# KrainskiL/CGE.jl

Measured on AMD Instinct MI355X. Metric: edge_alpha_evals_per_sec, higher is better.
Workload: dtype f64

## Files before the change

### cge.jl_amd/api.py

```python
from __future__ import annotations

import atexit
import ctypes as C
import os
import sys
import weakref

import numpy as np

from .args import _SplitRule

_HERE = os.path.dirname(os.path.abspath(__file__))
_LIB_PATH = os.path.join(_HERE, "csrc", "build", "libcge_hip.so")
_lib = None

CGE_OK = 0
_CODES = {-1: "AssertionError", -2: "ErrorException: Trying to split homogenous cluster",
          -3: "ErrorException: Unexpected empty cluster generated", -4: "HIP error / no GPU",
          -5: "collective hook failed", -6: "out of memory", -7: "bad argument"}


class CGEError(RuntimeError):
    def __init__(self, code, msg=""):
        super().__init__(f"{_CODES.get(code, 'error')} (code {code}){': ' + msg if msg else ''}")
# ... 817 lines not shown
        T, d = off.size - 1, self.d
        assert T >= 1 and off[0] == 0 and off[-1] == ids.size
        if z is not None:
            z = _f64(z)
            assert z.shape == ids.shape
        rc, nlow, children = np.zeros(T, dtype=np.int32), np.zeros(T, dtype=np.int32), np.full(ids.size, -1, dtype=np.int32)
        vlow, vhigh, cmeans = np.zeros(T), np.zeros(T), np.full((T, 2, d), np.nan)
        route, ties = np.zeros(T, dtype=np.int32), C.c_int32()
        self._check(self.L.cge_group_cut_test(self.h, _p(ids), _p(off), C.c_int64(T), C.c_int(int(method)), _p(z),
                                              C.c_int(1 if force_generic else 0), _p(rc), _p(nlow), _p(children), _p(vlow),
                                              _p(vhigh), _p(cmeans), _p(route), C.byref(ties)))
        return {"rc": rc, "nlow": nlow, "children": children, "vlow": vlow, "vhigh": vhigh, "cmeans": cmeans, "route": route,
                "ties": ties.value}

    def diameter_bounds_test(self, v_to_l, N, lcomm, C_, pass_):
        v2l, lc = _i64(v_to_l), _i64(lcomm)
        w = int(C_) if C_ >= 32 else int(N)
        P, ref, mean = np.zeros((N, w)), np.zeros((w, self.d)), np.zeros(self.d)
        nref, ran = C.c_int64(), C.c_int()
        self._check(self.L.cge_diameter_bounds_test(self.h, _p(v2l), C.c_int64(N), _p(lc), C.c_int64(C_), C.c_int(pass_), _p(P),
                                                    C.byref(nref), C.byref(ran), _p(ref), _p(mean)))
        assert nref.value == w
        return P, ran.value, ref, mean

    def landmark_graph_test(self, v_to_l, N, directed=False, wedge_form=0, part=0, nparts=1, aggregate=False, wedges=True,
                            positive=None, degrees=False, world=0):
        v2l = _i64(v_to_l)
        N = int(N)
        io, out = LandmarkGraphIO(), {}
        io.v2l, io.N, io.directed, io.wedge_form = v2l.ctypes.data, N, int(bool(directed)), int(wedge_form)
        io.part, io.nparts, io.world = int(part), int(nparts), int(world)

        def want(key, shape, dtype=np.float64):
            out[key] = np.full(shape, -1 if dtype != np.float64 else np.nan, dtype=dtype)
            setattr(io, key, out[key].ctypes.data)

        if aggregate:
            d = getattr(self, "d", 1)
            want("lemb", (N, d)), want("lweight", N), want("dii", N), want("lcomm", N, np.int32)
        positive = bool(wedges) if positive is None else positive
        if wedges:
            want("wedges", (N, N))
        if positive:
            want("positive", 1, np.int64)
        if degrees:
            want("deg_out", N), want("deg_in", N), want("star", N, np.int32)
# ... 334 lines not shown
                cap = count.value
                continue
            self._check(rc)
            break
        return [(comm[l], int(nc[l]), float(q[l]), int(rounds[l])) for l in range(count.value)]

    def ecg(self, members=16, w_min=0.05, seed=0, final_level=-1, edge_weights=False):
        args = EcgArgs(int(members), float(w_min), int(seed), int(final_level))
        out = np.zeros(self.n, dtype=np.int64)
        w = np.zeros(self.m) if edge_weights else None
        nc, q, q_ecg = C.c_int64(), C.c_double(), C.c_double()
        self._check(self.L.cge_ecg(self.h, C.byref(args), _p(out), C.byref(nc), C.byref(q), C.byref(q_ecg), _p(w) if edge_weights else None))
        return (out, nc.value, q.value, q_ecg.value) + ((w,) if edge_weights else ())

    def ecg_members_test(self, members=16, seed=0):
        K = int(members)
        mem = np.zeros((max(K, 1), self.n), dtype=np.int64)
        nc, rounds, q = np.zeros(max(K, 1), dtype=np.int64), np.zeros(max(K, 1), dtype=np.int64), np.zeros(max(K, 1))
        core = np.zeros(self.n, dtype=np.int32)
        self._check(self.L.cge_ecg_members_test(self.h, C.c_int64(K), C.c_int64(int(seed)), _p(mem), _p(nc), _p(rounds), _p(q), _p(core)))
        return mem, nc, rounds, q, core.astype(bool)

    _TEST_OPTIONS = ("louvain_wave_len", "fit_persistent_test_delay", "fit_persistent_test_timeout", "test_bvec_plain", "test_rss2_one_kernel",
                     "exact_resident_limit", "test_eig_roles", "fit_dir_tiles")

    def set_option(self, key, value):
        if key in self._TEST_OPTIONS:
            self._check(self.L.cge_set_test_option(self.h, key.encode(), C.c_int64(int(value))))
            return
        self._check(self.L.cge_set_option(self.h, key.encode(), C.c_int64(int(value))))

    def get_stat(self, key):
        v = C.c_int64()
        self._check(self.L.cge_get_stat(self.h, key.encode(), C.byref(v)))
        return v.value

    def last_diameter(self):
        import struct

        hi = struct.unpack("d", struct.pack("q", self.get_stat("diameter_bits")))[0]
        return hi, {1: "brute", 2: "pruned"}.get(self.get_stat("diameter_path"), "none"), \
            self.get_stat("diameter_candidate_pairs"), self.get_stat("diameter_candidate_tiles")

    def profile_enable(self, on=True):
        self._check(self.L.cge_profile_enable(self.h, C.c_int(int(on))))

    def profile_select(self, names=()):
# ... 126 lines not shown
```

### cge.jl_amd/csrc/capi.cpp

```cpp
#include "common.hpp"
#include "../../include/cge_hip_testing.h"

void flush_timers(cge_ctx *c) {
    for (auto &kv : c->timers) {
        for (auto &pr : kv.second.pending) {
            float ms = 0.f;
            (void)hipEventSynchronize(pr.second);
            if (hipEventElapsedTime(&ms, pr.first, pr.second) == hipSuccess) kv.second.total_ms += ms;
            c->event_pool.push_back(pr.first);
            c->event_pool.push_back(pr.second);
        }
        kv.second.pending.clear();
    }
}
template <class Map>
static int key_names(const Map &m, char *buf, int64_t buf_len) {
    std::string s;
    for (auto &kv : m) s += (s.empty() ? "" : ",") + kv.first;
    snprintf(buf, (size_t)buf_len, "%s", s.c_str());
    return CGE_OK;
}

extern "C" {

// ... 300 lines not shown
    if (is("fit_persistent")) return ranged(c->opt_fit_persistent, 0, 2);
    if (is("pow_exp2")) return flag(c->opt_pow_exp2);
    if (is("shard_runsplit")) return ranged(c->opt_shard_forced, 0, 2);
    if (is("shard_samples")) return ranged(c->opt_shard_samples, 0, 2);
    if (is("exact_relabel")) return flag(c->opt_exact_relabel);
    if (is("bvec_blocks")) return flag(c->opt_bvec_blocks);
    if (is("wedges_reduce_scatter")) return flag(c->opt_wedges_rs);
    if (is("fit_fused")) return flag(c->opt_fit_fused);
    if (is("shard_ingest")) return flag(c->opt_shard_ingest);
    if (is("shard_rows")) return flag(c->opt_shard_rows);
    if (is("landmark_edges")) return flag(c->opt_landmark_edges);
    if (is("exact_packed")) return ranged(c->opt_exact_packed, 0, 1);
    if (is("exact_packed_directed")) return ranged(c->opt_exact_packed_directed, 0, 2);
    if (is("fit_max_iterations")) return ranged(c->opt_fit_max_iters, 1, INT64_MAX);
    if (is("ecg_group")) return ranged(c->opt_ecg_group, 0, 64);
    return CGE_E_ARG;
}
int cge_set_test_option(void *ctx, const char *key, int64_t value) {
    cge_ctx *c = (cge_ctx *)ctx;
    if (!c || !key) return CGE_E_ARG;
    if (!strcmp(key, "test_bvec_plain")) { c->opt_test_bvec_plain = value != 0; return CGE_OK; }
    if (!strcmp(key, "test_rss2_one_kernel")) { c->opt_test_rss2_one_kernel = value != 0; return CGE_OK; }
    if (!strcmp(key, "test_eig_roles") && value >= 0 && value <= 3) { c->opt_test_eig_roles = (int)value; return CGE_OK; }
    if (!strcmp(key, "fit_persistent_test_delay") && value >= 0 && value <= 100000) { c->opt_fit_test_delay = (int)value; return CGE_OK; }
    if (!strcmp(key, "fit_persistent_test_timeout")) { c->opt_fit_test_timeout = value != 0; return CGE_OK; }
    if (!strcmp(key, "louvain_wave_len") && value >= -2 && value <= INT32_MAX) { c->opt_test_louvain_wave_len = value; return CGE_OK; }
    if (!strcmp(key, "fit_dir_tiles")) { c->opt_test_fit_dir_tiles = value != 0; return CGE_OK; }
    if (!strcmp(key, "exact_resident_limit") && value >= 0) { c->opt_test_resident_limit = (double)value; return CGE_OK; }
    return CGE_E_ARG;
}
int cge_get_stat(cge_ctx *c, const char *key, int64_t *value) {
    if (!c || !key || !value) return CGE_E_ARG;
    if (!strcmp(key, "landmarks")) *value = c->lm_ready ? c->N : 0;
    else if (!strcmp(key, "diameter_path")) *value = c->stat_diameter_path;
    else if (!strcmp(key, "diameter_candidate_pairs")) *value = c->stat_cand_pairs;
    else if (!strcmp(key, "diameter_candidate_tiles")) *value = c->stat_cand_tiles;
    else if (!strcmp(key, "diameter_refs")) *value = c->stat_nref;
    else if (!strcmp(key, "diameter_bound_pass")) *value = c->stat_bound_pass;
    else if (!strcmp(key, "diameter_arg_i")) *value = c->stat_hi_i + 1;
    else if (!strcmp(key, "diameter_arg_j")) *value = c->stat_hi_j + 1;
    else if (!strcmp(key, "fit_persistent_alphas")) *value = c->stat_fit_persistent;
    else if (!strcmp(key, "fit_iterations")) *value = c->stat_fit_iters;
    else if (!strcmp(key, "exact_packed")) *value = c->stat_exact_packed;
    else if (!strcmp(key, "exact_matrix_bytes")) *value = c->stat_exact_matrix_bytes;
    else if (!strcmp(key, "fit_fused_alphas")) *value = c->stat_fit_fused;
    else if (!strcmp(key, "fit_persistent_fallbacks")) *value = c->stat_fit_fallbacks;
// ... 133 lines not shown
    host_group_stats_test(c, ids, task_row_off, T, side, mean_in, mean, sw, cov, vec, z, sums);
    CGE_CATCH(c)
}

int cge_group_cut_test(void *ctx, const int32_t *ids, const int32_t *task_row_off, int64_t T, int method, const double *z, int force_generic,
                       int32_t *rc, int32_t *nlow, int32_t *children, double *vlow, double *vhigh, double *cmeans, int32_t *route,
                       int32_t *ties) {
    cge_ctx *c = (cge_ctx *)ctx;
    if (!c || !ids || !task_row_off || T <= 0 || !rc || !nlow || !children || !vlow || !vhigh || !cmeans || !route || !ties) return CGE_E_ARG;
    CGE_TRY_ON_DEVICE(c)
    host_group_cut_test(c, ids, task_row_off, T, method, z, force_generic, rc, nlow, children, vlow, vhigh, cmeans, route, ties);
    CGE_CATCH(c)
}

int cge_diameter_bounds_test(void *ctx, const int64_t *v2l, int64_t N, const int64_t *lcomm, int64_t C, int pass, double *P,
                             int64_t *nref, int *pass_ran, double *ref_points, double *mean) {
    cge_ctx *c = (cge_ctx *)ctx;
    if (!c || !v2l || !lcomm || !P || !nref || !pass_ran || N <= 0 || C <= 0 || pass < 0 || pass > 2) return CGE_E_ARG;
    CGE_TRY_ON_DEVICE(c)
    host_diameter_bounds_test(c, v2l, N, lcomm, C, pass, P, nref, pass_ran, ref_points, mean);
    CGE_CATCH(c)
}

int cge_landmark_graph_test(void *ctx, cge_landmark_graph_io *io) {
    cge_ctx *c = (cge_ctx *)ctx;
    if (!c || !io || !io->v2l || io->N <= 0 || io->wedge_form < 0 || io->wedge_form > 2) return CGE_E_ARG;
    CGE_TRY_ON_DEVICE(c)
    host_landmark_graph_test(c, io);
    CGE_CATCH(c)
}
int cge_wedge_geometry_test(int64_t N, int weighted, int64_t n_chunks, int *applies, int *rshift, int *colbits, int64_t *ntile,
                            int64_t *lds_pass1, int64_t *lds_pass2) {
    if (!applies || !rshift || !colbits || !ntile || !lds_pass1 || !lds_pass2) return CGE_E_ARG;
    WedgeGeometry G;
    *applies = k_wedge_geometry(N, weighted ? 8 : 4, n_chunks, &G) ? 1 : 0;
    if (!*applies) return CGE_OK;
    *rshift = G.rshift; *colbits = G.colbits; *ntile = G.ntile;
    *lds_pass1 = (int64_t)G.lds1; *lds_pass2 = (int64_t)G.lds2;
    return CGE_OK;
}

int cge_pow_test(void *ctx, const double *x, int64_t n, double alpha, int method, double *out) {
    cge_ctx *c = (cge_ctx *)ctx;
    if (!c || !x || !out || n <= 0) return CGE_E_ARG;
    CGE_TRY(c)
    k_pow_test(c, x, n, alpha, method, out);
// ... 143 lines not shown
```

### cge.jl_amd/csrc/common.hpp

```cpp
#pragma once
#include <hip/hip_runtime.h>

#include <algorithm>
#include <atomic>
#include <chrono>
#include <condition_variable>
#include <functional>
#include <mutex>
#include <thread>
#include <cstdint>
#include <cstdio>
#include <cstdlib>
#include <cstring>
#include <map>
#include <memory>
#include <string>
#include <vector>

#include "../../include/cge_hip.h"

typedef int64_t i64;
typedef int32_t i32;

struct MaxRec {
// ... 331 lines not shown
    DevBuf<double> sw_fused_pw;
    DevBuf<char> sw_fused_epi;
    int opt_fit_fused = 1;
    i64 stat_fit_fused = 0;
    DevBuf<double> batch_scal, batch_vectB, batch_jspart, batch_flow;
    PinBuf<double> batch_pin;
    i64 stat_fit_batched_launches = 0, stat_fit_batched_alphas = 0;
    DevBuf<i32> sw_rl_order, sw_rl_comm;
    DevBuf<double> sw_rl_emb, sw_rl_vec, sw_rl_T;
    DevBuf<int> fp_flags;
    PinBuf<double> pin_scal;
    hipEvent_t sweep_ev[2] = {nullptr, nullptr};
    int opt_pow_exp2 = 1;
    i64 pow_logs_N = 0;
    bool pow_logs_upper = false;
    i64 pow_logs_blocked_N = 0;
    DevBuf<double> sw_Lh;
    DevBuf<float> sw_Ll;
    bool opt_exact_relabel = true;
    int opt_shard_samples = 1;
    int opt_shard_forced = 1;
    int opt_test_rss2_one_kernel = 0;
    int opt_test_eig_roles = 0;
    i64 opt_test_louvain_wave_len = -2;
    int opt_ecg_group = 0;
    i64 stat_ecg_groups = 0, stat_ecg_member_rounds = 0, stat_ecg_peel_rounds = 0, stat_ecg_levels = 0;
    int opt_test_bvec_plain = 0;
    int opt_fit_persistent = 0;
    i64 opt_fit_max_iters = 2000000;
    int opt_fit_test_timeout = 0;
    int opt_fit_test_delay = 0;
    i64 stat_lm_batches = 0, stat_lm_rows = 0, stat_lm_splits = 0;
    DevBuf<int> cut_ties;
    i64 stat_fit_persistent = 0;
    i64 stat_fit_iters = 0;
    bool fit_persistent_broken = false;
    i64 stat_fit_fallbacks = 0;
    int fit_fallback_streak = 0;
    i64 fit_skip_sweeps = 0;
    DevBuf<i32> sw_cm_off, sw_cm_mem, sw_cm_pos;
    DevBuf<double> sw_zeros, sw_zsum;
    DevBuf<MaxRec> mp_recs;
    DevBuf<i64> mp_count;
    DevBuf<int2> nt_pairs, nt_tiles;
    DevBuf<i32> nt_idx;
    DevBuf<double> nt_out, nt_rows;
// ... 473 lines not shown
void k_js(cge_ctx *c, const double *vC, const double *vB, i64 len, i64 C, int directed, int mode ,
          double *out, double *partials = nullptr);
void k_auc_landmark(cge_ctx *c, const double *Ta, const double *Tb, const i32 *v2l, const double *vw_orig,
                    const double *lweight, const i32 *pi, const i32 *pj, const i32 *ni, const i32 *nj,
                    const double *dpos, const double *dneg, const double *wts, i64 S, double alpha, double *out2, double *partials = nullptr);
void k_auc_exact(cge_ctx *c, const double *GD, const double *Ta, const double *Tb, i64 N, const i32 *pi,
                 const i32 *pj, const i32 *ni, const i32 *nj, const double *wts, i64 S, double *out2, double *partials = nullptr,
                 bool packed = false);
void k_gather_i32(cge_ctx *c, const i32 *arr, const i32 *idx, i64 S, i32 *out);
void k_mark_edge_hits(cge_ctx *c, const i32 *src, const i32 *dst, i64 m, int directed, const uint64_t *table,
                      i64 table_size, i32 *hit);

void host_runsplit(cge_ctx *c, const i64 *cl_flat, const i64 *cl_off, i64 ncl, i64 nland, i64 forced, int method,
                   std::vector<i64> &group_ids , bool want_index = false);
void host_eig_top(const double *A, i64 d, double *v);
void host_group_stats_test(cge_ctx *c, const i32 *ids, const i32 *task_row_off, i64 T, const unsigned char *side, const double *mean_in,
                           double *mean, double *sw, double *cov, double *vec, double *z, double *sums);
void host_group_cut_test(cge_ctx *c, const i32 *ids, const i32 *task_row_off, i64 T, int method, const double *z, int force_generic,
                         i32 *rc, i32 *nlow, i32 *children, double *vlow, double *vhigh, double *cmeans, i32 *route, i32 *ties);
double host_diameter_brute(cge_ctx *c, int part, int nparts, i64 *ai, i64 *aj);
double host_diameter_landmarks(cge_ctx *c, const double *lemb, const double *lweight, const std::vector<i32> &lcomm, i64 C, i64 N);
void host_diameter_bounds_test(cge_ctx *c, const i64 *v2l, i64 N, const i64 *lcomm1, i64 C, int pass, double *P, i64 *nref_out,
                               int *pass_ran, double *ref_out, double *mean_out);
struct cge_landmark_graph_io;
void host_landmark_graph_test(cge_ctx *c, cge_landmark_graph_io *io);
#define CGE_TILE_DOUBLES 4096
__host__ __device__ inline i64 cge_upper_tile(i64 I, i64 J, i64 Nt) { return I * Nt - I * (I - 1) / 2 + (J - I); }
__host__ __device__ inline int cge_tile_slot(int r, int q) {
    const int lane = 8 * (r >> 3) + (q >> 3), a = r & 7, b = q & 7;
    return ((4 * a + (b >> 1)) * 64 + lane) * 2 + (b & 1);
}
__host__ __device__ inline i64 cge_packed_index(i64 i, i64 j, i64 Nt) {
    if ((i >> 6) > (j >> 6)) { const i64 s = i; i = j; j = s; }
    return cge_upper_tile(i >> 6, j >> 6, Nt) * CGE_TILE_DOUBLES + cge_tile_slot((int)(i & 63), (int)(j & 63));
}
__host__ __device__ inline void cge_upper_tile_of(i64 t, i64 Nt, i64 &I, i64 &J) {
    const double bb = 2.0 * (double)Nt + 1.0;
    I = (i64)((bb - sqrt(bb * bb - 8.0 * (double)t)) * 0.5);
    if (I < 0) I = 0;
    if (I > Nt - 1) I = Nt - 1;
    while (I + 1 < Nt && (I + 1) * Nt - (I + 1) * I / 2 <= t) I++;
    while (I > 0 && I * Nt - I * (I - 1) / 2 > t) I--;
    J = I + (t - (I * Nt - I * (I - 1) / 2));
}
__host__ __device__ inline uint64_t cge_sm64(uint64_t x) {
    x += 0x9e3779b97f4a7c15ULL;
// ... 118 lines not shown
```

### cge.jl_amd/csrc/diameter_host.cpp

```cpp
#include <algorithm>
#include <cmath>
#include <functional>
#include <limits>

#include "common.hpp"

namespace {
struct ExactBest {
    double hi = -1.0;
    i64 i = 0, j = 0;
    void offer(double v, i64 a, i64 b) {
        if (a > b) std::swap(a, b);
        if (v > hi || (v == hi && (a < i || (a == i && b < j)))) { hi = v; i = a; j = b; }
    }
};
struct SideStream {
    cge_ctx *c;
    explicit SideStream(cge_ctx *c_) : c(c_) { std::swap(c->stream, c->copy_stream); }
    ~SideStream() { std::swap(c->stream, c->copy_stream); }
};
}

static double gram_delta(i64 dpad, double rmax) { return (double)(8 * dpad + 32) * 2.220446049250313e-16 * rmax; }

// ... 560 lines not shown
        for (i64 q = mem_off[a]; q < mem_off[a + 1]; q++)
            for (i64 k = 0; k < d; k++) mu[a * d + k] += X[(i64)mem[q] * d + k];
        for (i64 k = 0; k < d; k++) mu[a * d + k] /= (double)cnt;
    }
    DevBuf<double> dmu, dlw;
    dmu.ensure((size_t)N * d);
    dlw.ensure(N);
    HIP_CHECK(hipMemcpyAsync(dmu.p, mu.data(), sizeof(double) * N * d, hipMemcpyHostToDevice, st));
    HIP_CHECK(hipMemcpyAsync(dlw.p, lw.data(), sizeof(double) * N, hipMemcpyHostToDevice, st));
    HIP_CHECK(hipStreamSynchronize(st));
    struct KeepOption { int &ref; int val; ~KeepOption() { ref = val; } } keep{c->opt_diameter_f32, c->opt_diameter_f32};
    c->opt_diameter_f32 = pass;
    DmPrep S;
    if (!dm_prepare(c, dmu.p, dlw.p, lc, C, N, mem_off, mem, S, [](const char *) {}))
        CGE_THROW(CGE_E_ARG, "diameter bounds: no landmark index");
    dm_bound_pass(c, S, N, 0, 1);
    HIP_CHECK(hipMemcpyAsync(P, c->Pm.p, sizeof(double) * (size_t)(N * S.nref), hipMemcpyDeviceToHost, st));
    if (ref_out) HIP_CHECK(hipMemcpyAsync(ref_out, S.mu_ref, sizeof(double) * (size_t)(S.nref * d), hipMemcpyDeviceToHost, st));
    if (mean_out) HIP_CHECK(hipMemcpyAsync(mean_out, c->gmean.p, sizeof(double) * d, hipMemcpyDeviceToHost, st));
    HIP_CHECK(hipStreamSynchronize(st));
    *nref_out = S.nref;
    *pass_ran = c->stat_bound_pass;
}
```

### cge.jl_amd/csrc/kernels_dist.hip

```cpp
#include "common.hpp"
#include <type_traits>
#include "mfma_tile.hpp"

#define WAVE 64

#define DT 64
#define DK 16
__device__ __forceinline__ void tile_dist2(const double *__restrict__ emb, i64 N, i64 d, i64 i0, i64 j0, int ty, int tx,
                                           double (*As)[DK + 1], double (*Bs)[DK + 1], double acc[4][4]) {
#pragma unroll
    for (int a = 0; a < 4; a++)
#pragma unroll
        for (int b = 0; b < 4; b++) acc[a][b] = 0.0;
    for (i64 k0 = 0; k0 < d; k0 += DK) {
        __syncthreads();
        for (int e = threadIdx.x; e < DT * DK; e += 256) {
            const int r = e / DK, kk = e % DK;
            const i64 k = k0 + kk;
            As[r][kk] = (i0 + r < N && k < d) ? emb[(i0 + r) * d + k] : 0.0;
            Bs[r][kk] = (j0 + r < N && k < d) ? emb[(j0 + r) * d + k] : 0.0;
        }
        __syncthreads();
        const int kmax = (int)min((i64)DK, d - k0);
        for (int kk = 0; kk < kmax; kk++) {
// ... 535 lines not shown
                            const i64 r0 = i0 + wr * 64 + a * 32 + 16 * h;
                            double v = -1e300;
#pragma unroll
                            for (int gg = 0; gg < 2; gg++)
#pragma unroll
                                for (int j = 0; j < 4; j++)
                                {
                            const float af = acc[a][b][4 * (2 * h + gg) + j];
                            v = fmax(v, (af - af == 0.f) ? rns[r0 + 8 * gg + 4 * lh + j] * e1 - 2.0 * (double)af : 1e300);
                        }
                            v = fmax(v, __shfl_xor(v, 32));
                            if (lh == 0) G[(r0 >> 4) * ldm + col] = fmax(v + mn, 0.0);
                        }
                }
            }
            __syncthreads();
        }
    }
}

typedef __bf16 bf8v __attribute__((ext_vector_type(8)));
typedef short s8v __attribute__((ext_vector_type(8)));
#define PB_APAD 8
#define PB_T 512
template <int NKS>
__global__ __launch_bounds__(PB_T) void pcent_bf16_kernel(const unsigned short *__restrict__ Xb, const double *__restrict__ rns,
                                                          i64 lds_rows, const unsigned short *__restrict__ Mb,
                                                          const double *__restrict__ mnorm, i64 ldm,
                                                          const i32 *__restrict__ sub_land, i64 nref,
                                                          unsigned long long *__restrict__ P, i64 I0, i64 I1, double e1,
                                                          int diag ) {
    extern __shared__ __attribute__((aligned(16))) unsigned short ldsb[];
    constexpr i64 KP = 16 * NKS;
    constexpr int LDA = (int)KP + PB_APAD;
    unsigned short *Ah = ldsb, *Al = Ah + (size_t)128 * LDA, *Bh = Al + (size_t)128 * LDA, *Bl = Bh + (size_t)128 * LDA;
    double *gmax = reinterpret_cast<double *>(Bl + (size_t)128 * LDA);
    const int tid = threadIdx.x, wave = tid >> 6, lane = tid & 63;
    const int wr = wave >> 1, wc = wave & 1, l32 = lane & 31, lh = lane >> 5;
    const i64 nTJ = ldm / 128;
    constexpr int apieces = (int)(KP / 8);
    const int arow = tid >> 5, apc = tid & 31;
    const bool aact = apc < 2 * apieces;
    const int apl = aact && apc >= apieces ? 1 : 0, akk = 8 * (apc - apl * apieces);
    auto fetch = [&](const unsigned short *base, i64 rows_ld, i64 r0, uint4 (&v)[8]) {
#pragma unroll
        for (int it = 0; it < 8; it++)
// ... 76 lines not shown
            __syncthreads();
            if (!(diag & 1) && tid < 128) {
                const i64 col = J * 128 + tid;
                double cur = 0.0;
                int curland = -1;
#pragma unroll
                for (int gq = 0; gq < 8; gq++) {
                    const int land = sub_land[(i0 >> 4) + gq];
                    const double v = gmax[gq * 128 + tid];
                    if (land != curland) {
                        if (curland >= 0 && col < nref) atomicMax(&P[(i64)curland * nref + col], (unsigned long long)__double_as_longlong(cur));
                        curland = land;
                        cur = v;
                    } else
                        cur = fmax(cur, v);
                }
                if (curland >= 0 && col < nref) atomicMax(&P[(i64)curland * nref + col], (unsigned long long)__double_as_longlong(cur));
            }
            if (more_cols) stash(Bh, Bl, bv);
            __syncthreads();
        }
    }
}
__global__ void pcent_groups_kernel(const double *__restrict__ G, const i32 *__restrict__ soff, i64 ldm, i64 N,
                                    double *__restrict__ P) {
    const i64 a = blockIdx.x;
    const i32 g0 = soff[a] >> 4, g1 = soff[a + 1] >> 4;
    for (i64 col = threadIdx.x; col < N; col += blockDim.x) {
        double v = 0.0;
        for (i32 g = g0; g < g1; g++) v = fmax(v, G[(i64)g * ldm + col]);
        P[a * N + col] = v;
    }
}

__global__ __launch_bounds__(256, 2) void pair_list_kernel(const double *__restrict__ Xs,
                                                           const double *__restrict__ rns, i64 lds_rows, i64 npos,
                                                           i64 dpad, const int2 *__restrict__ tiles, i64 ntiles,
                                                           MaxRec *__restrict__ recs) {
    extern __shared__ __attribute__((aligned(16))) double lds[];
    const int tid = threadIdx.x, wave = tid >> 6, lane = tid & 63;
    const int wr = wave >> 1, wc = wave & 1, lr = lane & 15, lk = lane >> 4, c2 = lane * 2;
    const i64 nchunk = dpad / MP_BK;
    double best = -1.0;
    i64 best_i = 0, best_j = 0;
    for (i64 t = blockIdx.x; t < ntiles; t += gridDim.x) {
        const i64 i0 = tiles[t].x, j0 = tiles[t].y;
// ... 99 lines not shown
    ScopedKernelTimer t(c, "pcent");
    const i64 nTI = lds_rows / 128, I0 = nTI * part / nparts, I1 = nTI * (part + 1) / nparts;
    const i64 ntiles = (I1 - I0) * (ldm / 128);
    const double e1 = 1.0 + 1.01 * (double)(dpad + 3) * 5.9604644775390625e-08;
    if (ntiles > 0 && dpad <= 128) {
        cge_allow_lds((const void *)pcent_f32_rowres_kernel, 160 * 1024);
        const size_t lds = ((size_t)dpad * 128 + 2 * PF_BK * 128) * sizeof(float);
        hipLaunchKernelGGL(pcent_f32_rowres_kernel, dim3((unsigned)std::min<i64>(I1 - I0, 512)), dim3(256), lds, c->stream, Xs32, rns,
                           lds_rows, Ms32, mnorm, ldm, N, dpad, c->pc_groups.p, I0, I1, e1);
    } else if (ntiles > 0)
        hipLaunchKernelGGL(pcent_f32_kernel, dim3((unsigned)std::min<i64>(ntiles, 2048)), dim3(256), PF_LDS_BYTES, c->stream,
                           Xs32, rns, lds_rows, Ms32, mnorm, ldm, N, dpad, c->pc_groups.p, I0, I1, e1);
    hipLaunchKernelGGL(pcent_groups_kernel, dim3((unsigned)n_land), dim3(256), 0, c->stream, c->pc_groups.p, soff, ldm, N, P);
}

bool k_pcent_bf16_applies(i64 dpad) { return (dpad + 31) / 32 * 32 <= 128; }
void k_pcent_bf16(cge_ctx *c, const unsigned short *Xb, const double *rns, i64 lds_rows, const unsigned short *Mb,
                  const double *mnorm, i64 ldm, i64 n_land, i64 N, i64 KP, const i32 *sub_land, double *P, int part, int nparts) {
    HIP_CHECK(hipMemsetAsync(P, 0, sizeof(double) * n_land * N, c->stream));
    ScopedKernelTimer t(c, "pcent");
    const i64 nTI = lds_rows / 128, I0 = nTI * part / nparts, I1 = nTI * (part + 1) / nparts;
    const double e1 = 1.0 + 1.05 * (3.0 * (double)(KP + 2) * 1.1920928955078125e-07 + 3.2 * 1.52587890625e-05);
    if (I1 > I0) {
        const size_t lds = (size_t)4 * 128 * (KP + PB_APAD) * sizeof(unsigned short) + (size_t)8 * 128 * sizeof(double);
        const int pb_diag = 0;
#define PB_GO(NKS)                                                                                                         \
    do {                                                                                                                   \
        auto kern = pcent_bf16_kernel<NKS>;                                                                                 \
        cge_allow_lds((const void *)kern, 160 * 1024); \
        hipLaunchKernelGGL(kern, dim3((unsigned)std::min<i64>(I1 - I0, 256)), dim3(PB_T), lds, c->stream, Xb, rns, lds_rows, Mb, \
                           mnorm, ldm, sub_land, N, reinterpret_cast<unsigned long long *>(P), I0, I1, e1, pb_diag);        \
    } while (0)
        if (KP == 32) PB_GO(2);
        else if (KP == 64) PB_GO(4);
        else if (KP == 96) PB_GO(6);
        else PB_GO(8);
#undef PB_GO
    }
}

void k_pair_list(cge_ctx *c, const double *Xs, const double *rns, i64 lds_rows, i64 npos, i64 dpad, const int2 *tiles,
                 i64 ntiles, double *best_val, i64 *best_i, i64 *best_j, std::vector<double> *wg_best) {
    c->mp_recs.ensure(MP_NWG);
    MaxRec *recs = c->mp_recs.p;
    const int nwg = (int)std::max<i64>(1, std::min<i64>(ntiles, MP_NWG));
    {
        ScopedKernelTimer t(c, "pair_list");
        hipLaunchKernelGGL(pair_list_kernel, dim3(nwg), dim3(256), MP_LDS_BYTES, c->stream, Xs, rns, lds_rows, npos,
                           dpad, tiles, ntiles, recs);
    }
    best_of_recs(c, recs, nwg, best_val, best_i, best_j, wg_best);
}

void k_max_pair_tile_list(i64 ldn, int part, int nparts, const std::vector<double> &wg, double thr, std::vector<int2> &out) {
// ... 25 lines not shown
    HIP_CHECK(hipStreamSynchronize(c->stream));
    return (i64)h;
}

__global__ __launch_bounds__(256) void bound_select_kernel(const double *__restrict__ Q, const i32 *__restrict__ lref,
                                                           const double *__restrict__ rd2, i64 N, i64 nref, double L,
                                                           BoundRec *__restrict__ list, i64 cap,
                                                           unsigned long long *__restrict__ count) {
    const i64 total = N * N, stride = (i64)gridDim.x * blockDim.x;
    for (i64 e = (i64)blockIdx.x * blockDim.x + threadIdx.x; e < total; e += stride) {
        const i64 a = e / N, b = e - a * N;
        if (b < a) continue;
        const i64 ra = lref[a], rb = lref[b];
        const double qaa = Q[a * nref + ra], qbb = Q[b * nref + rb];
        const double pre = Q[a * nref + rb] + Q[b * nref + ra] + 2.0 * sqrt(qaa * qbb);
        if (pre * (1.0 + 1e-9) + 1e-9 < L) continue;
        const double Bv = pre - rd2[ra * nref + rb] * (1.0 - 1e-9);
        if (Bv * (1.0 + 1e-9) + 1e-9 >= L) {
            const unsigned long long idx = atomicAdd(count, 1ULL);
            if ((i64)idx < cap) list[idx] = BoundRec{Bv, (i32)a, (i32)b};
        }
    }
}
__global__ __launch_bounds__(256) void ref_dist2_fm_kernel(const double *__restrict__ Ms, i64 nref, i64 dpad, i64 ldm,
                                                           double *__restrict__ rd2) {
    const i64 a = blockIdx.x;
    for (i64 b = threadIdx.x; b < nref; b += blockDim.x) {
        double s = 0.0;
#pragma unroll 8
        for (i64 k = 0; k < dpad; k++) {
            const double df = Ms[k * ldm + a] - Ms[k * ldm + b];
            s += df * df;
        }
        rd2[a * nref + b] = s;
    }
}
__global__ __launch_bounds__(256) void comm_max_kernel(const double *__restrict__ Q, const i32 *__restrict__ ref_off,
                                                       const i32 *__restrict__ ref_mem, i64 nref, double *__restrict__ Mx) {
    const i64 ca = blockIdx.x;
    const i32 b = ref_off[ca], e = ref_off[ca + 1];
    for (i64 r = threadIdx.x; r < nref; r += blockDim.x) {
        double v = 0.0;
        for (i32 t = b; t < e; t++) v = fmax(v, Q[(i64)ref_mem[t] * nref + r]);
        Mx[ca * nref + r] = v;
    }
}
__global__ __launch_bounds__(256) void comm_pairs_kernel(const double *__restrict__ Mx, const double *__restrict__ rd2, i64 C,
                                                         double L, int2 *__restrict__ plist, unsigned *__restrict__ pcount) {
    const i64 total = C * C, stride = (i64)gridDim.x * blockDim.x;
    for (i64 e = (i64)blockIdx.x * blockDim.x + threadIdx.x; e < total; e += stride) {
        const i64 ca = e / C, cb = e - ca * C;
        if (cb < ca) continue;
        const double pre = Mx[ca * C + cb] + Mx[cb * C + ca] + 2.0 * sqrt(Mx[ca * C + ca] * Mx[cb * C + cb]);
        if (pre * (1.0 + 1e-9) + 1e-9 < L) continue;
        const double Bv = pre - rd2[ca * C + cb] * (1.0 - 1e-9);
        if (Bv * (1.0 + 1e-9) + 1e-9 >= L) plist[atomicAdd(pcount, 1u)] = make_int2((int)ca, (int)cb);
    }
// ... 7 lines not shown
    for (unsigned q = blockIdx.x; q < np; q += gridDim.x) {
        const i64 ca = plist[q].x, cb = plist[q].y;
        const i32 a0 = ref_off[ca], na = ref_off[ca + 1] - a0, b0 = ref_off[cb], nb = ref_off[cb + 1] - b0;
        const double r2 = rd2[ca * nref + cb] * (1.0 - 1e-9);
        for (i64 e = threadIdx.x; e < (i64)na * nb; e += blockDim.x) {
            const i64 ia = e / nb, ib = e - ia * nb;
            i64 a = ref_mem[a0 + ia], b = ref_mem[b0 + ib];
            if (ca == cb && b < a) continue;
            i64 ra = ca, rb = cb;
            if (b < a) { const i64 t = a; a = b; b = t; ra = cb; rb = ca; }
            const double qaa = Q[a * nref + ra], qbb = Q[b * nref + rb];
            const double pre = Q[a * nref + rb] + Q[b * nref + ra] + 2.0 * sqrt(qaa * qbb);
            if (pre * (1.0 + 1e-9) + 1e-9 < L) continue;
            const double Bv = pre - r2;
            if (Bv * (1.0 + 1e-9) + 1e-9 >= L) {
                const unsigned long long idx = atomicAdd(count, 1ULL);
                if ((i64)idx < cap) list[idx] = BoundRec{Bv, (i32)a, (i32)b};
            }
        }
    }
}
void k_ref_dist2_fm(cge_ctx *c, const double *Ms_fm, i64 nref, i64 dpad, i64 ldm) {
    c->mp_rd2.ensure((size_t)nref * nref);
    hipLaunchKernelGGL(ref_dist2_fm_kernel, dim3((unsigned)nref), dim3(256), 0, c->stream, Ms_fm, nref, dpad, ldm, c->mp_rd2.p);
}
i64 k_bound_select(cge_ctx *c, const double *Q, const i32 *lref, i64 N, i64 nref, double L, BoundRec *list, i64 cap,
                   const i32 *ref_off, const i32 *ref_mem) {
    c->mp_count.ensure(2);
    HIP_CHECK(hipMemsetAsync(c->mp_count.p, 0, 2 * sizeof(i64), c->stream));
    ScopedKernelTimer tm(c, "bound_select");
    if (ref_off && ref_mem) {
        c->mp_commax.ensure((size_t)nref * nref);
        c->mp_plist.ensure((size_t)nref * (nref + 1) / 2);
        hipLaunchKernelGGL(comm_max_kernel, dim3((unsigned)nref), dim3(256), 0, c->stream, Q, ref_off, ref_mem, nref, c->mp_commax.p);
        hipLaunchKernelGGL(comm_pairs_kernel, dim3(grid_for(nref * nref, 256)), dim3(256), 0, c->stream, c->mp_commax.p, c->mp_rd2.p,
                           nref, L, c->mp_plist.p, reinterpret_cast<unsigned *>(c->mp_count.p + 1));
        hipLaunchKernelGGL(bound_expand_kernel, dim3(2048), dim3(256), 0, c->stream, Q, c->mp_rd2.p, ref_off, ref_mem, nref, L,
                           c->mp_plist.p, reinterpret_cast<const unsigned *>(c->mp_count.p + 1), list, cap,
                           reinterpret_cast<unsigned long long *>(c->mp_count.p));
    } else
        hipLaunchKernelGGL(bound_select_kernel, dim3(grid_for(N * N, 256)), dim3(256), 0, c->stream, Q, lref, c->mp_rd2.p, N,
                           nref, L, list, cap, reinterpret_cast<unsigned long long *>(c->mp_count.p));
    i64 cnt = 0;
    HIP_CHECK(hipMemcpyAsync(&cnt, c->mp_count.p, sizeof(i64), hipMemcpyDeviceToHost, c->stream));
    HIP_CHECK(hipStreamSynchronize(c->stream));
    return cnt;
}
// ... 208 lines not shown
```

### include/cge_hip_testing.h

```cpp
#ifndef CGE_HIP_TESTING_H
#define CGE_HIP_TESTING_H
#include <stdint.h>
#ifdef __cplusplus
extern "C" {
#endif
int cge_host_eig_top(const double *A, int64_t d, double *v);
int cge_batch_pack_test(const int64_t *N, int64_t K, int cus, int32_t *group_of);
int cge_fit_dir_geometry_test(int64_t N, int cus, int *applies, int *G, int *NW, int *NSB);
int cge_fit_slots_test(int64_t N, int directed, int64_t out[5]);
int cge_batch_pack_dir_test(const int64_t *N, int64_t K, int cus, int32_t *group_of);
int cge_host_pos_draw(int64_t seed, int64_t stream_id, int64_t S, int64_t m, int64_t *pos_idx);
int cge_group_eig(void *ctx, const double *A, int64_t T, int64_t d, double *v);
int cge_group_stats_test(void *ctx, const int32_t *ids, const int32_t *task_row_off, int64_t T, const uint8_t *side, const double *mean_in,
                         double *mean, double *sw, double *cov, double *vec, double *z, double *sums);
int cge_group_cut_test(void *ctx, const int32_t *ids, const int32_t *task_row_off, int64_t T, int method, const double *z, int force_generic,
                       int32_t *rc, int32_t *nlow, int32_t *children, double *vlow, double *vhigh, double *cmeans, int32_t *route,
                       int32_t *ties);
int cge_diameter_bounds_test(void *ctx, const int64_t *v2l, int64_t N, const int64_t *lcomm, int64_t C, int pass, double *P,
                             int64_t *nref, int *pass_ran, double *ref_points, double *mean);
typedef struct cge_landmark_graph_io {
    const int64_t *v2l;
    int64_t N;
    int32_t directed, wedge_form;
    int64_t part, nparts, world;
    double *lemb, *lweight, *dii;
    int32_t *lcomm;
    double *wedges;
    int64_t *positive;
    double *deg_out, *deg_in;
    int32_t *star;
    double *deg_block, *u_deg_out, *u_deg_in;
    int32_t *u_star;
    int64_t n_chunks, ntile;
    int32_t form_ran, rshift, colbits, pad;
} cge_landmark_graph_io;
int cge_landmark_graph_test(void *ctx, cge_landmark_graph_io *io);
int cge_wedge_geometry_test(int64_t N, int weighted, int64_t n_chunks, int *applies, int *rshift, int *colbits, int64_t *ntile,
                            int64_t *lds_pass1, int64_t *lds_pass2);
int cge_pow_test(void *ctx, const double *x, int64_t n, double alpha, int method, double *out);
#define CGE_VECT_B_GUARD 64
typedef struct cge_vect_b_problem {
    const double *GD, *Ta, *Tb;
// ... 108 lines not shown
```

Baseline: 11.96 billion.

## Add register-resident B-tile pcent kernel and tiled reference distance kernel

Adds a pcent_bf16 kernel variant that keeps the reference (B) fragments in registers per wave across many row tiles, with a double-buffered prefetch of A tiles through LDS. It is selected by default when ldm is at least 384. The reference pairwise-distance kernel is also rewritten as a 32x32 shared-memory tiled kernel instead of one block per row. Both aim to cut repeated global/LDS reads of the reference matrix, at the cost of higher register pressure and a separate code path. The change also adds test hooks for selecting the pcent form and for reference distances.

```diff
diff --git a/cge.jl_amd/api.py b/cge.jl_amd/api.py
--- a/cge.jl_amd/api.py
+++ b/cge.jl_amd/api.py
@@ -863,6 +863,14 @@
                                                     C.byref(nref), C.byref(ran), _p(ref), _p(mean)))
         assert nref.value == w
         return P, ran.value, ref, mean
+
+    def ref_dist2_test(self, refs):
+        refs = _f64(refs)
+        assert refs.ndim == 2 and refs.shape[1] == self.d
+        nref = refs.shape[0]
+        rd2, mean = np.zeros((nref, nref)), np.zeros(self.d)
+        self._check(self.L.cge_ref_dist2_test(self.h, _p(refs), C.c_int64(nref), _p(rd2), _p(mean)))
+        return rd2, mean
 
     def landmark_graph_test(self, v_to_l, N, directed=False, wedge_form=0, part=0, nparts=1, aggregate=False, wedges=True,
                             positive=None, degrees=False, world=0):
@@ -1243,7 +1251,7 @@
         return mem, nc, rounds, q, core.astype(bool)
 
     _TEST_OPTIONS = ("louvain_wave_len", "fit_persistent_test_delay", "fit_persistent_test_timeout", "test_bvec_plain", "test_rss2_one_kernel",
-                     "exact_resident_limit", "test_eig_roles", "fit_dir_tiles")
+                     "exact_resident_limit", "test_eig_roles", "fit_dir_tiles", "test_pcent_form")
 
     def set_option(self, key, value):
         if key in self._TEST_OPTIONS:
diff --git a/cge.jl_amd/csrc/capi.cpp b/cge.jl_amd/csrc/capi.cpp
--- a/cge.jl_amd/csrc/capi.cpp
+++ b/cge.jl_amd/csrc/capi.cpp
@@ -346,6 +346,7 @@
     if (!strcmp(key, "test_bvec_plain")) { c->opt_test_bvec_plain = value != 0; return CGE_OK; }
     if (!strcmp(key, "test_rss2_one_kernel")) { c->opt_test_rss2_one_kernel = value != 0; return CGE_OK; }
     if (!strcmp(key, "test_eig_roles") && value >= 0 && value <= 3) { c->opt_test_eig_roles = (int)value; return CGE_OK; }
+    if (!strcmp(key, "test_pcent_form") && value >= 0 && value <= 2) { c->opt_test_pcent_form = (int)value; return CGE_OK; }
     if (!strcmp(key, "fit_persistent_test_delay") && value >= 0 && value <= 100000) { c->opt_fit_test_delay = (int)value; return CGE_OK; }
     if (!strcmp(key, "fit_persistent_test_timeout")) { c->opt_fit_test_timeout = value != 0; return CGE_OK; }
     if (!strcmp(key, "louvain_wave_len") && value >= -2 && value <= INT32_MAX) { c->opt_test_louvain_wave_len = value; return CGE_OK; }
@@ -525,6 +526,14 @@
     CGE_CATCH(c)
 }
 
+int cge_ref_dist2_test(void *ctx, const double *refs, int64_t nref, double *rd2, double *mean) {
+    cge_ctx *c = (cge_ctx *)ctx;
+    if (!c || !refs || !rd2 || nref <= 0) return CGE_E_ARG;
+    CGE_TRY_ON_DEVICE(c)
+    host_ref_dist2_test(c, refs, nref, rd2, mean);
+    CGE_CATCH(c)
+}
+
 int cge_landmark_graph_test(void *ctx, cge_landmark_graph_io *io) {
     cge_ctx *c = (cge_ctx *)ctx;
     if (!c || !io || !io->v2l || io->N <= 0 || io->wedge_form < 0 || io->wedge_form > 2) return CGE_E_ARG;
diff --git a/cge.jl_amd/csrc/common.hpp b/cge.jl_amd/csrc/common.hpp
--- a/cge.jl_amd/csrc/common.hpp
+++ b/cge.jl_amd/csrc/common.hpp
@@ -377,6 +377,7 @@
     int opt_shard_forced = 1;
     int opt_test_rss2_one_kernel = 0;
     int opt_test_eig_roles = 0;
+    int opt_test_pcent_form = 0;
     i64 opt_test_louvain_wave_len = -2;
     int opt_ecg_group = 0;
     i64 stat_ecg_groups = 0, stat_ecg_member_rounds = 0, stat_ecg_peel_rounds = 0, stat_ecg_levels = 0;
@@ -896,6 +897,7 @@
 double host_diameter_landmarks(cge_ctx *c, const double *lemb, const double *lweight, const std::vector<i32> &lcomm, i64 C, i64 N);
 void host_diameter_bounds_test(cge_ctx *c, const i64 *v2l, i64 N, const i64 *lcomm1, i64 C, int pass, double *P, i64 *nref_out,
                                int *pass_ran, double *ref_out, double *mean_out);
+void host_ref_dist2_test(cge_ctx *c, const double *refs, i64 nref, double *rd2, double *mean_out);
 struct cge_landmark_graph_io;
 void host_landmark_graph_test(cge_ctx *c, cge_landmark_graph_io *io);
 #define CGE_TILE_DOUBLES 4096
diff --git a/cge.jl_amd/csrc/diameter_host.cpp b/cge.jl_amd/csrc/diameter_host.cpp
--- a/cge.jl_amd/csrc/diameter_host.cpp
+++ b/cge.jl_amd/csrc/diameter_host.cpp
@@ -606,3 +606,21 @@
     *nref_out = S.nref;
     *pass_ran = c->stat_bound_pass;
 }
+
+void host_ref_dist2_test(cge_ctx *c, const double *refs, i64 nref, double *rd2, double *mean_out) {
+    const i64 d = c->d, dpad = c->dpad;
+    if (!c->Xr.p || c->n <= 0 || d <= 0) CGE_THROW(CGE_E_ARG, "reference distances: embedding not resident");
+    hipStream_t st = c->stream;
+    const i64 ldm = (nref + 127) / 128 * 128;
+    DevBuf<double> dref;
+    dref.ensure((size_t)nref * d);
+    HIP_CHECK(hipMemcpyAsync(dref.p, refs, sizeof(double) * nref * d, hipMemcpyHostToDevice, st));
+    HIP_CHECK(hipStreamSynchronize(st));
+    c->Ms.ensure((size_t)ldm * dpad);
+    c->mnorm.ensure(ldm);
+    k_gather_centre_fm(c, dref.p, nullptr, c->gmean.p, c->Ms.p, c->mnorm.p, nref, d, ldm, dpad, nullptr, nullptr, (dpad + 31) / 32 * 32, nullptr);
+    k_ref_dist2_fm(c, c->Ms.p, nref, dpad, ldm);
+    HIP_CHECK(hipMemcpyAsync(rd2, c->mp_rd2.p, sizeof(double) * (size_t)(nref * nref), hipMemcpyDeviceToHost, st));
+    if (mean_out) HIP_CHECK(hipMemcpyAsync(mean_out, c->gmean.p, sizeof(double) * d, hipMemcpyDeviceToHost, st));
+    HIP_CHECK(hipStreamSynchronize(st));
+}
diff --git a/cge.jl_amd/csrc/kernels_dist.hip b/cge.jl_amd/csrc/kernels_dist.hip
--- a/cge.jl_amd/csrc/kernels_dist.hip
+++ b/cge.jl_amd/csrc/kernels_dist.hip
@@ -581,6 +581,7 @@
 typedef __bf16 bf8v __attribute__((ext_vector_type(8)));
 typedef short s8v __attribute__((ext_vector_type(8)));
 #define PB_APAD 8
+#define PB_REG_MIN_LDM 384
 #define PB_T 512
 template <int NKS>
 __global__ __launch_bounds__(PB_T) void pcent_bf16_kernel(const unsigned short *__restrict__ Xb, const double *__restrict__ rns,
@@ -703,6 +704,150 @@
         }
     }
 }
+template <int NKS>
+__global__ __launch_bounds__(PB_T) void pcent_bf16_reg_kernel(const unsigned short *__restrict__ Xb, const double *__restrict__ rns,
+                                                              i64 lds_rows, const unsigned short *__restrict__ Mb,
+                                                              const double *__restrict__ mnorm, i64 ldm,
+                                                              const i32 *__restrict__ sub_land, i64 nref,
+                                                              unsigned long long *__restrict__ P, i64 I0, i64 I1, double e1) {
+    extern __shared__ __attribute__((aligned(16))) unsigned short ldsb[];
+    constexpr i64 KP = 16 * NKS;
+    constexpr int LDA = (int)KP + PB_APAD;
+    constexpr size_t ABUF = (size_t)2 * 128 * LDA;
+    double *rnl = reinterpret_cast<double *>(ldsb + 2 * ABUF);
+    const int tid = threadIdx.x, wave = tid >> 6, lane = tid & 63, l32 = lane & 31, lh = lane >> 5;
+    constexpr int apieces = (int)(KP / 8);
+    const int arow = tid >> 5, apc = tid & 31;
+    const bool aact = apc < 2 * apieces;
+    const int apl = aact && apc >= apieces ? 1 : 0, akk = 8 * (apc - apl * apieces);
+    uint4 av[4];
+    double rv = 0.0;
+    const size_t aoff = ((size_t)apl * lds_rows + arow) * KP + akk;
+    auto fetch = [&](i64 r0, int half) {
+        const unsigned short *px = Xb + (r0 + 64 * half) * KP + aoff;
+#pragma unroll
+        for (int it = 0; it < 4; it++)
+            av[it] = aact ? *reinterpret_cast<const uint4 *>(px + (size_t)16 * it * KP) : make_uint4(0, 0, 0, 0);
+        if (half == 0 && tid < 128) rv = rns[r0 + tid];
+    };
+    auto stash = [&](int s, int half) {
+        if (aact) {
+#pragma unroll
+            for (int it = 0; it < 4; it++)
+                *reinterpret_cast<uint4 *>(ldsb + s * ABUF + (size_t)apl * 128 * LDA + (size_t)(64 * half + 16 * it + arow) * LDA + akk) = av[it];
+        }
+        if (half == 0 && tid < 128) rnl[s * 128 + tid] = rv * e1;
+    };
+    const i64 step = gridDim.x;
+    for (i64 c0 = 0; c0 < ldm; c0 += 512) {
+        const i64 cb = c0 + 64 * wave;
+        const bool own = cb < ldm;
+        s8v bh[2][NKS], bl[2][NKS];
+        double mne[2];
+#pragma unroll
+        for (int b = 0; b < 2; b++) {
+            const size_t ob = (size_t)(own ? cb + b * 32 + l32 : 0) * KP + 8 * lh;
+#pragma unroll
+            for (int ks = 0; ks < NKS; ks++) {
+                bh[b][ks] = *reinterpret_cast<const s8v *>(Mb + ob + 16 * ks);
+                bl[b][ks] = *reinterpret_cast<const s8v *>(Mb + (size_t)ldm * KP + ob + 16 * ks);
+            }
+            mne[b] = mnorm[own ? cb + b * 32 + l32 : 0] * e1;
+        }
+        i64 I = I0 + blockIdx.x;
+        asm volatile("" : "+s"(I));
+        if (I < I1) {
+            fetch(I * 128, 0);
+            stash(0, 0);
+            fetch(I * 128, 1);
+            stash(0, 1);
+        }
+        if (I + step < I1) fetch((I + step) * 128, 0);
+        __syncthreads();
+        for (int s = 0; I < I1; I += step, s ^= 1) {
+            const bool more = I + step < I1;
+            const unsigned short *Ah = ldsb + s * ABUF, *Al = Ah + (size_t)128 * LDA;
+            const double *rn = rnl + s * 128;
+            const i32 *sl = sub_land + ((I * 128) >> 4);
+            int curland = -1;
+            double cur[2] = {0.0, 0.0};
+            auto flush = [&]() {
+                if (curland >= 0 && lh == 0) {
+#pragma unroll
+                    for (int b = 0; b < 2; b++) {
+                        const i64 col = cb + b * 32 + l32;
+                        if (col < nref) atomicMax(&P[(i64)curland * nref + col], (unsigned long long)__double_as_longlong(cur[b]));
+                    }
+                }
+            };
+#pragma unroll 1
+            for (int rb = 0; rb < 4; rb++) {
+                if (own) {
+                    f16v acc[2];
+#pragma unroll
+                    for (int b = 0; b < 2; b++)
+#pragma unroll
+                        for (int r = 0; r < 16; r++) acc[b][r] = 0.f;
+                    const size_t oa = (size_t)(rb * 32 + l32) * LDA + 8 * lh;
+                    s8v ah = *reinterpret_cast<const s8v *>(Ah + oa), al = *reinterpret_cast<const s8v *>(Al + oa);
+#pragma unroll
+                    for (int ks = 0; ks < NKS; ks++) {
+                        s8v nh = ah, nl = al;
+                        if (ks + 1 < NKS) {
+                            nh = *reinterpret_cast<const s8v *>(Ah + oa + 16 * (ks + 1));
+                            nl = *reinterpret_cast<const s8v *>(Al + oa + 16 * (ks + 1));
+                        }
+#pragma unroll
+                        for (int b = 0; b < 2; b++) {
+                            acc[b] = __builtin_amdgcn_mfma_f32_32x32x16_bf16(__builtin_bit_cast(bf8v, ah), __builtin_bit_cast(bf8v, bh[b][ks]), acc[b], 0, 0, 0);
+                            acc[b] = __builtin_amdgcn_mfma_f32_32x32x16_bf16(__builtin_bit_cast(bf8v, ah), __builtin_bit_cast(bf8v, bl[b][ks]), acc[b], 0, 0, 0);
+                            acc[b] = __builtin_amdgcn_mfma_f32_32x32x16_bf16(__builtin_bit_cast(bf8v, al), __builtin_bit_cast(bf8v, bh[b][ks]), acc[b], 0, 0, 0);
+                        }
+                        __builtin_amdgcn_sched_barrier(0);
+                        ah = nh;
+                        al = nl;
+                    }
+#pragma unroll
+                    for (int h = 0; h < 2; h++) {
+                        const int land = sl[rb * 2 + h];
+                        double v[2] = {-1e300, -1e300};
+#pragma unroll
+                        for (int q = 0; q < 8; q++) {
+                            const double rq = rn[rb * 32 + 16 * h + 8 * (q >> 2) + 4 * lh + (q & 3)];
+#pragma unroll
+                            for (int b = 0; b < 2; b++) {
+                                const float af = acc[b][8 * h + q];
+                                const double t = rq - 2.0 * (double)af;
+                                v[b] = fmax(v[b], (af - af == 0.f) ? t : 1e300);
+                            }
+                        }
+                        const bool fresh = land != curland;
+                        if (fresh) {
+                            flush();
+                            curland = land;
+                        }
+#pragma unroll
+                        for (int b = 0; b < 2; b++) {
+                            double w = fmax(v[b], __shfl_xor(v[b], 32));
+                            w = fmax(w + mne[b], 0.0);
+                            cur[b] = fresh ? w : fmax(cur[b], w);
+                        }
+                    }
+                }
+                if (more && rb == 1) {
+                    stash(s ^ 1, 0);
+                    fetch((I + step) * 128, 1);
+                }
+            }
+            if (own) flush();
+            if (more) {
+                stash(s ^ 1, 1);
+                if (I + 2 * step < I1) fetch((I + 2 * step) * 128, 0);
+            }
+            __syncthreads();
+        }
+    }
+}
 __global__ void pcent_groups_kernel(const double *__restrict__ G, const i32 *__restrict__ soff, i64 ldm, i64 N,
                                     double *__restrict__ P) {
     const i64 a = blockIdx.x;
@@ -848,14 +993,23 @@
     const i64 nTI = lds_rows / 128, I0 = nTI * part / nparts, I1 = nTI * (part + 1) / nparts;
     const double e1 = 1.0 + 1.05 * (3.0 * (double)(KP + 2) * 1.1920928955078125e-07 + 3.2 * 1.52587890625e-05);
     if (I1 > I0) {
-        const size_t lds = (size_t)4 * 128 * (KP + PB_APAD) * sizeof(unsigned short) + (size_t)8 * 128 * sizeof(double);
+        const bool reg = c->opt_test_pcent_form == 2 || (c->opt_test_pcent_form == 0 && ldm >= PB_REG_MIN_LDM);
+        const size_t lds = (size_t)4 * 128 * (KP + PB_APAD) * sizeof(unsigned short) + (size_t)(reg ? 2 : 8) * 128 * sizeof(double);
         const int pb_diag = 0;
+        const dim3 grid((unsigned)std::min<i64>(I1 - I0, 256));
+        unsigned long long *Pu = reinterpret_cast<unsigned long long *>(P);
 #define PB_GO(NKS)                                                                                                         \
     do {                                                                                                                   \
-        auto kern = pcent_bf16_kernel<NKS>;                                                                                 \
-        cge_allow_lds((const void *)kern, 160 * 1024); \
-        hipLaunchKernelGGL(kern, dim3((unsigned)std::min<i64>(I1 - I0, 256)), dim3(PB_T), lds, c->stream, Xb, rns, lds_rows, Mb, \
-                           mnorm, ldm, sub_land, N, reinterpret_cast<unsigned long long *>(P), I0, I1, e1, pb_diag);        \
+        if (reg) {                                                                                                         \
+            auto kern = pcent_bf16_reg_kernel<NKS>;                                                                        \
+            cge_allow_lds((const void *)kern, 160 * 1024);                                                                 \
+            hipLaunchKernelGGL(kern, grid, dim3(PB_T), lds, c->stream, Xb, rns, lds_rows, Mb, mnorm, ldm, sub_land, N, Pu, I0, I1, e1); \
+        } else {                                                                                                           \
+            auto kern = pcent_bf16_kernel<NKS>;                                                                            \
+            cge_allow_lds((const void *)kern, 160 * 1024);                                                                 \
+            hipLaunchKernelGGL(kern, grid, dim3(PB_T), lds, c->stream, Xb, rns, lds_rows, Mb, mnorm, ldm, sub_land, N, Pu, I0, I1, e1, \
+                               pb_diag);                                                                                   \
+        }                                                                                                                  \
     } while (0)
         if (KP == 32) PB_GO(2);
         else if (KP == 64) PB_GO(4);
@@ -927,17 +1081,36 @@
         }
     }
 }
+#define RD_T 32
+#define RD_KC 64
 __global__ __launch_bounds__(256) void ref_dist2_fm_kernel(const double *__restrict__ Ms, i64 nref, i64 dpad, i64 ldm,
                                                            double *__restrict__ rd2) {
-    const i64 a = blockIdx.x;
-    for (i64 b = threadIdx.x; b < nref; b += blockDim.x) {
-        double s = 0.0;
-#pragma unroll 8
-        for (i64 k = 0; k < dpad; k++) {
-            const double df = Ms[k * ldm + a] - Ms[k * ldm + b];
-            s += df * df;
-        }
-        rd2[a * nref + b] = s;
+    __shared__ double As[RD_KC * RD_T], Bs[RD_KC * RD_T];
+    const i64 a0 = (i64)blockIdx.y * RD_T, b0 = (i64)blockIdx.x * RD_T;
+    const int tb = threadIdx.x & 31, ta = threadIdx.x >> 5;
+    double s[4] = {0.0, 0.0, 0.0, 0.0};
+    for (i64 k0 = 0; k0 < dpad; k0 += RD_KC) {
+        const int kc = dpad - k0 < RD_KC ? (int)(dpad - k0) : RD_KC;
+        if (k0) __syncthreads();
+        for (int kk = ta; kk < kc; kk += 8) {
+            As[kk * RD_T + tb] = Ms[(k0 + kk) * ldm + a0 + tb];
+            Bs[kk * RD_T + tb] = Ms[(k0 + kk) * ldm + b0 + tb];
+        }
+        __syncthreads();
+#pragma unroll 4
+        for (int kk = 0; kk < kc; kk++) {
+            const double vb = Bs[kk * RD_T + tb];
+#pragma unroll
+            for (int j = 0; j < 4; j++) {
+                const double df = As[kk * RD_T + ta + 8 * j] - vb;
+                s[j] += df * df;
+            }
+        }
+    }
+#pragma unroll
+    for (int j = 0; j < 4; j++) {
+        const i64 a = a0 + ta + 8 * j, b = b0 + tb;
+        if (a < nref && b < nref) rd2[a * nref + b] = s[j];
     }
 }
 __global__ __launch_bounds__(256) void comm_max_kernel(const double *__restrict__ Q, const i32 *__restrict__ ref_off,
@@ -991,7 +1164,8 @@
 }
 void k_ref_dist2_fm(cge_ctx *c, const double *Ms_fm, i64 nref, i64 dpad, i64 ldm) {
     c->mp_rd2.ensure((size_t)nref * nref);
-    hipLaunchKernelGGL(ref_dist2_fm_kernel, dim3((unsigned)nref), dim3(256), 0, c->stream, Ms_fm, nref, dpad, ldm, c->mp_rd2.p);
+    const unsigned nt = (unsigned)((nref + RD_T - 1) / RD_T);
+    hipLaunchKernelGGL(ref_dist2_fm_kernel, dim3(nt, nt), dim3(256), 0, c->stream, Ms_fm, nref, dpad, ldm, c->mp_rd2.p);
 }
 i64 k_bound_select(cge_ctx *c, const double *Q, const i32 *lref, i64 N, i64 nref, double L, BoundRec *list, i64 cap,
                    const i32 *ref_off, const i32 *ref_mem) {
diff --git a/include/cge_hip_testing.h b/include/cge_hip_testing.h
--- a/include/cge_hip_testing.h
+++ b/include/cge_hip_testing.h
@@ -18,6 +18,7 @@
                        int32_t *ties);
 int cge_diameter_bounds_test(void *ctx, const int64_t *v2l, int64_t N, const int64_t *lcomm, int64_t C, int pass, double *P,
                              int64_t *nref, int *pass_ran, double *ref_points, double *mean);
+int cge_ref_dist2_test(void *ctx, const double *refs, int64_t nref, double *rd2, double *mean);
 typedef struct cge_landmark_graph_io {
     const int64_t *v2l;
     int64_t N;
```

New measurement: 12.16 billion, median of 6. 1.02x the previous value.
